# yjh0410/YOLO-Nano

Hardware: AMD Instinct MI355X
Metric: images/sec YOLO-Nano-1.0x 416x416 bs=32 inference (network + decode + NMS + host delivery) (higher is better)
Workload: dtype f32 (split-f16 MFMA x3, fp32 accumulate); 1 GPU; YOLO-Nano-1.0x 416x416 bs=32/GPU fp32 inference, COCO 80-class head + NMS (BASELINE configs[1]); inputs resident in HBM, kept detections delivered to pinned host memory inside the timed region; global_batch=32, parallelism=image-sharded x1, no collective, rccl_ranks=1, launch_mode=eager, streams_per_gpu=4

## Files before the change

include/yolonano_hip.h:

```cpp
#ifndef YOLONANO_HIP_H
#define YOLONANO_HIP_H

#include <stdint.h>

#ifdef __cplusplus
extern "C" {
#endif

typedef struct yn_handle yn_handle;

enum { YN_BACKBONE_0_5X = 0, YN_BACKBONE_1_0X = 1, YN_BACKBONE_1_5X = 2, YN_BACKBONE_2_0X = 3 };
enum { YN_ACT_NONE = 0, YN_ACT_RELU = 1, YN_ACT_LEAKY = 2 };
enum { YN_F32 = 0, YN_F16 = 1 };
enum { YN_STATUS_OK = 0, YN_STATUS_ERROR = 1, YN_STATUS_RANGE = 2 };

typedef struct yn_config {
    int   input_size;
    int   num_classes;
    int   num_anchors;
    float anchors[18];
    int   backbone;
    float conf_thresh;
    float nms_thresh;
    int   diou_nms;
// ... 166 lines not shown
int  yn_train_get_loss_scale(yn_handle* h, float* scale, float* clean_steps);
int  yn_train_set_loss_scale(yn_handle* h, float scale, float clean_steps);
int  yn_allreduce_grads(yn_handle* h, void* nccl_comm);
int  yn_train_forward(yn_handle* h, const float* x_dev, int B, float* head_s8_dev, float* head_s16_dev, float* head_s32_dev);
int  yn_train_skipped_steps(yn_handle* h, int64_t* count_host);
int  yn_train_head_fork(yn_handle* h, int force, int* decision_host);
int  yn_train_precision(yn_handle* h, int dtype);
int  yn_train_graph(yn_handle* h, int enable, int64_t* replays);

int  yn_op_dwconv3x3(yn_handle* h, const float* x, int B, int H, int W, int C, int stride,
                     const float* w, const float* bias, int act, float* y);
int  yn_op_pwconv(yn_handle* h, const float* x, int B, int H, int W, int Cin, int Cout,
                  const float* w, const float* bias, int act, float* y);
int  yn_op_pwconv_shuffle(yn_handle* h, const float* x, const float* pass, int B, int H, int W, int Cin, int Cout,
                          const float* w, const float* bias, int act, float* y);
int  yn_op_conv3x3(yn_handle* h, const float* x, const float* x2, int resample, int B, int H, int W,
                   int Cin, int Cout, const float* w, const float* bias, int act, float* y);
int  yn_op_stem(yn_handle* h, const float* x_nchw, int B, int H, int W, int Cout,
                const float* w, const float* bias, int act, float* y);
int  yn_op_stem_pool(yn_handle* h, const float* x_nchw, int B, int H, int W, int Cout,
                     const float* w, const float* bias, int act, float* y);
int  yn_op_maxpool3x3s2(yn_handle* h, const float* x, int B, int H, int W, int C, float* y);
int  yn_op_shuffle_block(yn_handle* h, const char* block, const float* x, int B, int H, int W, float* y);
int  yn_op_nchw_to_nhwc(yn_handle* h, const float* x, int B, int C, int H, int W, float* y);
int  yn_op_nhwc_to_nchw(yn_handle* h, const float* x, int B, int C, int H, int W, float* y);

int  yn_op_h16_conv(yn_handle* h, int kind, const float* x, int B, int H, int W, int Cin, int gapped, const float* w, const float* bias,
                    int Cout, int stride, const float* dy, float* y, float* dx, float* dw);
int  yn_op_h16_conv2(yn_handle* h, int kind, const float* x, int B, int H, int W, int Cin, int gapped, int x_ld, int x_off,
                     const float* w, const float* bias, int Cout, int stride, const float* dy, int accumulate, int dx_ld, int dx_off,
                     int64_t partial_cap, int stat, const float* y_below, const float* mean, const float* invstd, const float* gamma,
                     const float* beta, int act, float* y, float* dx, float* dw, float* dbias, double* sums_fwd, double* sums_bwd);
int  yn_op_h16_stem(yn_handle* h, const float* x_nchw, int B, int H, int W, const float* w, const float* bias, const float* dy, float* y, float* dw);
int  yn_op_h16_maxpool(yn_handle* h, const float* x, int B, int H, int W, int C, const float* dy, float* y, uint8_t* idx, float* dx);
int  yn_op_h16_stem_pool(yn_handle* h, const float* y, int B, int H, int W, const float* gamma, const float* beta, int act, const float* g1,
                         float* out, uint8_t* idx, float* mean, float* invstd, float* dy, float* dgamma, float* dbeta);
int  yn_op_h16_resample(yn_handle* h, int mode, const float* a, const float* b, float* out, int B, int H, int W, int C);
int  yn_op_h16_gather(yn_handle* h, const float* src, int src_ld, int src_off, int src_cs, int src_half, int src_gap,
                      float* dst, int dst_ld, int dst_off, int dst_cs, int dst_half, int dst_gap, int64_t M, int n, int npad);
int  yn_op_h16_grad_finish(yn_handle* h, float* g, const float* slots, int64_t n, float* state, int update, int global_flag);
int  yn_op_h16_loss(yn_handle* h, const float* head_s8, const float* head_s16, const float* head_s32, const float* target, int B, float scale,
                    float* losses, float* g_s8, float* g_s16, float* g_s32, int* pad_nonzero);
int  yn_op_h16_gemm_stats(yn_handle* h, int kind, const float* x, int B, int H, int W, int Cin, int gapped, const float* w, int Cout,
                          float* y, double* sums_fwd, const float* dy, const float* y_below, const float* mean, const float* invstd,
                          const float* gamma, const float* beta, int act, float* dx, double* sums_bwd);
int  yn_op_h16_bn(yn_handle* h, const float* y, const float* dz, int64_t M, int C, const float* gamma, const float* beta, int act,
// ... 50 lines not shown
```

yolo-nano_amd/capi.py:

```python
import ctypes
import os

import numpy as np
import torch

from . import arch

_HERE = os.path.dirname(os.path.abspath(__file__))
LIB_PATH = os.path.join(_HERE, "libyolonano_hip.so")

_vp = ctypes.c_void_p
_i32, _f32 = ctypes.c_int, ctypes.c_float
_i64p = ctypes.POINTER(ctypes.c_int64)

BACKBONE_ID = {"0.5x": 0, "1.0x": 1, "1.5x": 2, "2.0x": 3}


class YnConfig(ctypes.Structure):
    _fields_ = [("input_size", _i32), ("num_classes", _i32), ("num_anchors", _i32),
                ("anchors", _f32 * 18), ("backbone", _i32), ("conf_thresh", _f32), ("nms_thresh", _f32),
                ("diou_nms", _i32), ("max_batch", _i32), ("device", _i32), ("stream", _vp)]


SIGNATURES = {
# ... 52 lines not shown
    "yn_train_forward": (_i32, [_vp, _vp, _i32, _vp, _vp, _vp]),
    "yn_train_skipped_steps": (_i32, [_vp, _i64p]),
    "yn_train_head_fork": (_i32, [_vp, _i32, ctypes.POINTER(ctypes.c_int)]),
    "yn_train_precision": (_i32, [_vp, _i32]),
    "yn_train_graph": (_i32, [_vp, _i32, _vp]),
    "yn_train_get_loss_scale": (_i32, [_vp, ctypes.POINTER(_f32), ctypes.POINTER(_f32)]),
    "yn_train_set_loss_scale": (_i32, [_vp, _f32, _f32]),
    "yn_make_targets": (_i32, [_vp, _vp, _vp, _i32, _vp, _vp]),
    "yn_preprocess": (_i32, [_vp, _vp, _i32, _i32, _i32, _i32, _i32, _i32, _i32, _vp, _vp, _vp]),
    "yn_preprocess_batch": (_i32, [_vp, _i32, _vp, _vp, _i32, _vp, _vp, _vp]),
    "yn_train_transform_batch": (_i32, [_vp, _i32, _vp, _vp, _vp, _i32, _vp, _vp, _vp]),
    "yn_mosaic_transform_batch": (_i32, [_vp, _i32, _vp, _vp, _vp, _i32, _i32, _vp, _vp, _vp]),
    "yn_nms_merge": (_i32, [_vp, _vp, _vp, _vp, _i32, _i32, _f32, _i32, _vp, _vp, _vp, _vp, _vp]),
    "yn_ema_update": (_i32, [_vp, _vp, _vp, ctypes.c_int64, ctypes.c_double]),
    "yn_sgd_step": (_i32, [_vp, _vp, _vp, _vp, ctypes.c_int64, _f32, _f32, _f32, _f32, _i32]),
    "yn_op_dwconv3x3": (_i32, [_vp, _vp, _i32, _i32, _i32, _i32, _i32, _vp, _vp, _i32, _vp]),
    "yn_op_pwconv": (_i32, [_vp, _vp, _i32, _i32, _i32, _i32, _i32, _vp, _vp, _i32, _vp]),
    "yn_op_pwconv_shuffle": (_i32, [_vp, _vp, _vp, _i32, _i32, _i32, _i32, _i32, _vp, _vp, _i32, _vp]),
    "yn_op_conv3x3": (_i32, [_vp, _vp, _vp, _i32, _i32, _i32, _i32, _i32, _i32, _vp, _vp, _i32, _vp]),
    "yn_op_stem": (_i32, [_vp, _vp, _i32, _i32, _i32, _i32, _vp, _vp, _i32, _vp]),
    "yn_op_stem_pool": (_i32, [_vp, _vp, _i32, _i32, _i32, _i32, _vp, _vp, _i32, _vp]),
    "yn_op_maxpool3x3s2": (_i32, [_vp, _vp, _i32, _i32, _i32, _i32, _vp]),
    "yn_op_shuffle_block": (_i32, [_vp, ctypes.c_char_p, _vp, _i32, _i32, _i32, _vp]),
    "yn_op_nchw_to_nhwc": (_i32, [_vp, _vp, _i32, _i32, _i32, _i32, _vp]),
    "yn_op_nhwc_to_nchw": (_i32, [_vp, _vp, _i32, _i32, _i32, _i32, _vp]),
    "yn_op_h16_conv": (_i32, [_vp, _i32, _vp, _i32, _i32, _i32, _i32, _i32, _vp, _vp, _i32, _i32, _vp, _vp, _vp, _vp]),
    "yn_op_h16_conv2": (_i32, [_vp, _i32, _vp, _i32, _i32, _i32, _i32, _i32, _i32, _i32, _vp, _vp, _i32, _i32, _vp, _i32, _i32, _i32, ctypes.c_int64,
                               _i32, _vp, _vp, _vp, _vp, _vp, _i32, _vp, _vp, _vp, _vp, _vp, _vp]),
    "yn_op_h16_stem": (_i32, [_vp, _vp, _i32, _i32, _i32, _vp, _vp, _vp, _vp, _vp]),
    "yn_op_h16_maxpool": (_i32, [_vp, _vp, _i32, _i32, _i32, _i32, _vp, _vp, _vp, _vp]),
    "yn_op_h16_stem_pool": (_i32, [_vp, _vp, _i32, _i32, _i32, _vp, _vp, _i32, _vp, _vp, _vp, _vp, _vp, _vp, _vp, _vp]),
    "yn_op_h16_resample": (_i32, [_vp, _i32, _vp, _vp, _vp, _i32, _i32, _i32, _i32]),
    "yn_op_h16_gather": (_i32, [_vp, _vp, _i32, _i32, _i32, _i32, _i32, _vp, _i32, _i32, _i32, _i32, _i32, ctypes.c_int64, _i32, _i32]),
    "yn_op_h16_grad_finish": (_i32, [_vp, _vp, _vp, ctypes.c_int64, _vp, _i32, _i32]),
    "yn_op_h16_loss": (_i32, [_vp, _vp, _vp, _vp, _vp, _i32, _f32, _vp, _vp, _vp, _vp, ctypes.POINTER(_i32)]),
    "yn_op_h16_bn2": (_i32, [_vp, _vp, _vp, ctypes.c_int64, _i32, _vp, _vp, _i32, _vp, _vp, _vp, _vp, _vp, _vp]),
    "yn_op_h16_bn": (_i32, [_vp, _vp, _vp, ctypes.c_int64, _i32, _vp, _vp, _i32, _vp, _vp, _vp, _vp]),
    "yn_op_h16_gemm_stats": (_i32, [_vp, _i32, _vp, _i32, _i32, _i32, _i32, _i32, _vp, _i32, _vp, _vp, _vp, _vp, _vp, _vp, _vp, _vp, _i32, _vp, _vp]),
    "yn_op_h16_bn_unit": (_i32, [_vp, _vp, _vp, _vp, ctypes.c_int64, _i32, _vp, _vp, _i32, _vp, _vp, _vp, _vp, _vp]),
    "yn_op_f32_conv": (_i32, [_vp, _i32, _vp, _i32, _i32, _i32, _i32, _i32, _i32, _vp, _vp, _i32, _i32, _i32, ctypes.c_int64, _vp, _i32, _vp, _vp, _vp, _vp]),
    "yn_op_f32_bn": (_i32, [_vp, _vp, ctypes.c_int64, _i32, _vp, _vp, _i32, _i32, _vp, _vp, _vp, _vp, _vp, _vp, _vp, _i32, _i32, _vp, _vp, _vp, _vp]),
    "yn_op_f32_maxpool": (_i32, [_vp, _vp, _i32, _i32, _i32, _i32, _vp, _vp, _vp, _vp]),
    "yn_op_f32_resample": (_i32, [_vp, _i32, _vp, _vp, _vp, _i32, _i32, _i32, _i32]),
    "yn_eval_create": (_i32, [_vp, _i32, ctypes.c_double, ctypes.POINTER(_vp)]),
    "yn_eval_destroy": (None, [_vp]),
    "yn_eval_reset": (_i32, [_vp, _vp]),
# ... 638 lines not shown
        return y

    def op_stem_pool(self, x_nchw, w, bias, act=0):
        B, _, H, W = x_nchw.shape
        Cout = w.shape[0]
        Hc, Wc = (H - 1) // 2 + 1, (W - 1) // 2 + 1
        y = torch.empty((B, (Hc - 1) // 2 + 1, (Wc - 1) // 2 + 1, Cout), dtype=torch.float32, device=x_nchw.device)
        self._ck(self.lib.yn_op_stem_pool(self.h, _ptr(self._in(x_nchw)), B, H, W, Cout, _ptr(self._in(w)),
                                          _ptr(self._in(bias)) if bias is not None else None, act, y.data_ptr()), "yn_op_stem_pool")
        return y

    def op_maxpool(self, x):
        B, H, W, C = x.shape
        y = torch.empty((B, (H - 1) // 2 + 1, (W - 1) // 2 + 1, C), dtype=torch.float32, device=x.device)
        self._ck(self.lib.yn_op_maxpool3x3s2(self.h, _ptr(self._in(x)), B, H, W, C, y.data_ptr()), "yn_op_maxpool3x3s2")
        return y

    def op_shuffle_block(self, block, x, cout, stride):
        B, H, W, _ = x.shape
        y = torch.empty((B, (H - 1) // stride + 1, (W - 1) // stride + 1, cout), dtype=torch.float32, device=x.device)
        self._ck(self.lib.yn_op_shuffle_block(self.h, block.encode(), _ptr(self._in(x)), B, H, W, y.data_ptr()), "yn_op_shuffle_block")
        return y

    def op_h16_conv(self, kind, x, w, bias=None, stride=1, dy=None, gapped=False):
        B, H, W, Cin = x.shape
        Cout = w.shape[0]
        Ho, Wo = (H - 1) // stride + 1, (W - 1) // stride + 1
        y = torch.empty((B, Ho, Wo, Cout), dtype=torch.float32, device=x.device)
        dx = torch.empty_like(x) if dy is not None else None
        dw = torch.empty_like(w) if dy is not None else None
        self._ck(self.lib.yn_op_h16_conv(self.h, int(kind), self._in(x).data_ptr(), B, H, W, Cin, int(bool(gapped)), self._in(w).data_ptr(), _ptr(bias),
                                         Cout, int(stride), _ptr(self._in(dy) if dy is not None else None), y.data_ptr(), _ptr(dx), _ptr(dw)), "yn_op_h16_conv")
        return y, dx, dw

    def op_h16_bn(self, y, gamma, beta, act=0, dz=None):
        M, C = y.shape
        z = torch.empty_like(y)
        dy = torch.empty_like(y) if dz is not None else None
        dg = torch.empty((C,), dtype=torch.float32, device=y.device) if dz is not None else None
        db = torch.empty((C,), dtype=torch.float32, device=y.device) if dz is not None else None
        self._ck(self.lib.yn_op_h16_bn(self.h, self._in(y).data_ptr(), _ptr(self._in(dz) if dz is not None else None), M, C, gamma.data_ptr(), beta.data_ptr(),
                                       int(act), z.data_ptr(), _ptr(dy), _ptr(dg), _ptr(db)), "yn_op_h16_bn")
        return z, dy, dg, db

    def op_h16_bn2(self, y, gamma, beta, act=0, dz=None):
        M, C = y.shape
# ... 278 lines not shown
```

yolo-nano_amd/csrc/kernels_chain.hip:

```cpp
#include "yn_internal.h"
#include "yn_device.h"

#include <cstdlib>

namespace ynk {

template <int WM, int WN, int NT, int V>
__global__ __launch_bounds__(256, 2) void unit_chain_kernel(ChainArgs a)
{
    typedef typename VecT<V>::type vec;
    constexpr int BM = 32 * WM, BN = 32 * NT * WN, KP = 16, BS = BN * 2, B_PER = KP * BN / 512, G = V / 2;
    constexpr int MAXB = (BM * (BN / (2 * G)) + 255) / 256;
    static_assert(WM * WN == 4 && B_PER >= 1, "4 waves");
    extern __shared__ __attribute__((aligned(16))) float uc_smem[];
    const int bf = a.bf, CS = bf + 2, W = a.W, H = a.H, HW = H * W;
    float* T = uc_smem;
    float* Bs = uc_smem + ((BM * CS + 3) & ~3);

    const int t = threadIdx.x, lane = t & 63, wave = t >> 6, l31 = lane & 31, h = lane >> 5;
    const int wm = wave % WM, wn = wave / WM;
    const int m0 = (int)xcd_block(blockIdx.x, gridDim.x) * BM;
    if (m0 >= a.M) return;
    const int nchunks = (bf + 2 * KP - 1) / (2 * KP), kp_total = bf >> 1;

// ... 530 lines not shown
    if (a.Ws2h) {
        if (!dry && launch_unit_pipe(a, s)) return true;
        if (a.Npad == 64 && !v4) YN_UC2(2, 2, 1, 2, 4)
        if (a.Npad == 64 && v4) YN_UC2(2, 2, 1, 4, 4)
        constexpr int small_m = 4096;
        if (a.Npad == 128 && v4 && a.M <= small_m) YN_UC2(1, 4, 1, 4, 4)
        if (a.Npad == 128 && v4) YN_UC2(2, 2, 2, 4, 3)
        if (a.Npad == 256 && v4) YN_UC2(1, 4, 2, 4, 3)
        if (a.Npad == 32 && v4) YN_UC2(4, 1, 1, 4, 4)
        if (a.Npad == 96 && v4) YN_UC2(4, 1, 3, 4, 2)
        return false;
    }
#undef YN_UC2
    const int tiles64 = (a.M + 63) / 64;
    if (a.Npad == 64 && !v4) YN_UC(2, 2, 1, 2)
    if (a.Npad == 64 && v4) YN_UC(2, 2, 1, 4)
    if (a.Npad == 128 && v4) YN_UC(2, 2, 2, 4)
    if (a.Npad == 256 && v4) { if (tiles64 >= 256) YN_UC(2, 2, 4, 4) else YN_UC(1, 4, 2, 4) }
    if (a.Npad == 32 && v4) YN_UC(4, 1, 1, 4)
    if (a.Npad == 96 && v4) YN_UC(4, 1, 3, 4)
#undef YN_UC
    return false;
}
template <int NP, bool RELU>
__global__ __launch_bounds__(256, 2) void down_unit_pipe_kernel(DownArgs a, int tiles)
{
    constexpr int TW = 8, TH = 4, WW = 2 * TW + 1, WH = 2 * TH + 1, NPIX = WW * WH, RT1 = (NPIX + 31) / 32;
    constexpr int BN = 32 * NP, AST1 = 32 + 8, AST2 = BN + 8, NO = TW * TH, NLD = 5, KS2 = 2 * NP;
    extern __shared__ __attribute__((aligned(16))) float du_smem[];
    const int bf = a.bf, CS = bf + 2, cin = a.cin, cq = cin >> 2;
    h16* A1h = reinterpret_cast<h16*>(du_smem);
    h16* A1l = A1h + RT1 * 32 * AST1;
    h16* A2h = A1h;
    h16* A2l = A2h + NO * AST2;
    h16* A3h = A2l + NO * AST2;
    h16* A3l = A3h + NO * AST1;
    float* X32 = du_smem + RT1 * 32 * AST1;
    float* T32 = X32 + RT1 * 32 * cin;
    unsigned char* inside = reinterpret_cast<unsigned char*>(T32 + RT1 * 32 * CS);

    const int t = threadIdx.x, lane = t & 63, wave = __builtin_amdgcn_readfirstlane(t >> 6), l31 = lane & 31, h = lane >> 5;
    const int Ho = a.H >> 1, Wo = a.W >> 1;
    const int tx_n = (Wo + TW - 1) / TW, ty_n = (Ho + TH - 1) / TH, per_img = tx_n * ty_n;
    const int KQ1 = (cin + 7) >> 3, KQ2 = (bf + 7) >> 3;
    const int TL = (tiles + 7) >> 3, GL = (int)(gridDim.x >> 3);
    const int tbase = (int)(blockIdx.x & 7u) * TL;
    int tl = (int)(blockIdx.x >> 3);
    if (tl >= TL || tbase + tl >= tiles) return;
    auto act_pw = [&](float v, int act) { return RELU ? __builtin_fmaxf(v, 0.0f) : apply_act(v, act); };

#ifdef YN_EXP_TIMING
    long long TS[8]; int tsn = 0;
#define YN_TS() if (tsn < 8) TS[tsn++] = __builtin_readcyclecounter()
#else
#define YN_TS()
#endif
    YN_TS();
    const int cp_n = bf >> 1, ppl = 256 / cp_n;
    const int cp = t % cp_n, dpl = t / cp_n, dc = cp * 2;
    const bool dworker = dpl < ppl;
    float2 wd[9], bd = make_float2(0.0f, 0.0f);
#pragma unroll
    for (int k = 0; k < 9; ++k) wd[k] = dworker ? *reinterpret_cast<const float2*>(a.wdw + k * bf + dc) : make_float2(0.0f, 0.0f);
    if (dworker) bd = *reinterpret_cast<const float2*>(a.bdw + dc);
    const int c1_n = cin >> 1, p1_n = 256 / c1_n;
    const int c1 = (t % c1_n) * 2, p1 = t / c1_n;
    constexpr int NI1 = 2;
    float2 w1d[9], b1d;
#pragma unroll
    for (int k = 0; k < 9; ++k) w1d[k] = *reinterpret_cast<const float2*>(a.wdw1 + k * cin + c1);
    b1d = *reinterpret_cast<const float2*>(a.bdw1 + c1);
    const int it0 = 3 - wave;
    const int nt1 = (NP == 2) ? (it0 & 1) : 0;
    const bool pw2_wave = wave < NP, b1_wave = wave >= NP && wave < 2 * NP;
    const int nt2 = pw2_wave ? wave : wave - NP;
    auto frag = [&](const void* Wh_, const void* Wl_, int ks, int KQ, int n, bool use, h16x8& bh, h16x8& bl) {
        const int kq = ks * 2 + h;
        const bool ok = use && kq < KQ;
        const size_t off = ((size_t)(ok ? kq : 0) * BN + (ok ? n : 0)) * 8;
        const unsigned mk = opaque_mask(ok);
        uint4 vh = *reinterpret_cast<const uint4*>(reinterpret_cast<const h16*>(Wh_) + off), vl = *reinterpret_cast<const uint4*>(reinterpret_cast<const h16*>(Wl_) + off);
        vh.x &= mk; vh.y &= mk; vh.z &= mk; vh.w &= mk; vl.x &= mk; vl.y &= mk; vl.z &= mk; vl.w &= mk;
        bh = *reinterpret_cast<h16x8*>(&vh); bl = *reinterpret_cast<h16x8*>(&vl);
    };
    h16x8 g1h[2], g1l[2], g2h[KS2], g2l[KS2];
#pragma unroll
    for (int ks = 0; ks < 2; ++ks) frag(a.W1h, a.W1l, ks, KQ1, nt1 * 32 + l31, true, g1h[ks], g1l[ks]);
#pragma unroll
    for (int ks = 0; ks < KS2; ++ks) {
        const bool use = pw2_wave || (b1_wave && ks < 2);
        frag(pw2_wave ? a.W2h : a.W3h, pw2_wave ? a.W2l : a.W3l, ks, pw2_wave ? KQ2 : KQ1, nt2 * 32 + l31, use, g2h[ks], g2l[ks]);
    }
    const float bias1 = (nt1 * 32 + l31 < bf) ? a.b1[nt1 * 32 + l31] : 0.0f;
    const float bias23 = (nt2 * 32 + l31 < bf && (pw2_wave || b1_wave)) ? (pw2_wave ? a.b2 : a.b3)[nt2 * 32 + l31] : 0.0f;
    const int QR = WW * cq;
    int wpos[NLD], wrel[NLD];
#pragma unroll
    for (int i = 0; i < NLD; ++i) {
        const int e = t + 256 * i;
        const int wy = e / QR, q = e - wy * QR;
        const int wx = q / cq, c4 = (q - wx * cq) * 4;
        wpos[i] = (e < WH * QR) ? (wy | (wx << 8) | (c4 << 16)) : -1;
        wrel[i] = (wy * a.W + wx) * cin + c4;
    }
    float4 pre[NLD];
    unsigned pok = 0;
    const char* xbase = reinterpret_cast<const char*>(a.x);
    auto request = [&](int tile) {
        const int b = tile / per_img, trem = tile - b * per_img;
        const int ty = trem / tx_n, tx = trem - ty * tx_n;
        const int iy0 = 2 * ty * TH - 1, ix0 = 2 * tx * TW - 1;
        const int org = ((b * a.H + iy0) * a.W + ix0) * cin;
        pok = 0;
#pragma unroll
        for (int i = 0; i < NLD; ++i) {
            const int wy = wpos[i] & 0xff, wx = (wpos[i] >> 8) & 0xff;
            const bool ok = wpos[i] >= 0 && (unsigned)(iy0 + wy) < (unsigned)a.H && (unsigned)(ix0 + wx) < (unsigned)a.W;
            pre[i] = *reinterpret_cast<const float4*>(xbase + (unsigned)(ok ? org + wrel[i] : 0) * 4u);
// ... 2 lines not shown
    };
    request(tbase + tl);
    if (t < RT1 * 32 - NPIX) inside[NPIX + t] = 0;
    float amax = 0.0f;
    float* PT = T32;

    auto consume = [&]() {
#pragma unroll
        for (int i = 0; i < NLD; ++i) {
            if (wpos[i] >= 0) {
                const int wy = wpos[i] & 0xff, wx = (wpos[i] >> 8) & 0xff, c4 = (wpos[i] >> 16) & 0xff;
                const int p = wy * WW + wx;
                const float4 v = vmask(pre[i], 0u - ((pok >> i) & 1u));
                *reinterpret_cast<float4*>(X32 + p * cin + c4) = v;
                const float x4[4] = {v.x, v.y, v.z, v.w};
                h16x4 hi, lo;
#pragma unroll
                for (int j = 0; j < 4; ++j) { amax = range_track(amax, x4[j]); hi[j] = (h16)x4[j]; lo[j] = split_lo(x4[j], hi[j]); }
                *reinterpret_cast<h16x4*>(A1h + p * AST1 + c4) = hi;
                *reinterpret_cast<h16x4*>(A1l + p * AST1 + c4) = lo;
                if (c4 == 0) inside[p] = (unsigned char)((pok >> i) & 1u);
            }
        }
        {
            const int ntail = (32 - cin) >> 2;
            for (int i = t; i < RT1 * 32 * ntail; i += 256) {
                const int p = i / ntail, c2 = cin + 4 * (i - p * ntail);
                *reinterpret_cast<uint2*>(A1h + p * AST1 + c2) = make_uint2(0u, 0u);
                *reinterpret_cast<uint2*>(A1l + p * AST1 + c2) = make_uint2(0u, 0u);
            }
        }
    };
    consume();

    for (;;) {
        const int tile = tbase + tl;
        const int b = tile / per_img, trem = tile - b * per_img;
        const int oy0 = (trem / tx_n) * TH, ox0 = (trem % tx_n) * TW;
        __syncthreads();
        YN_TS();
        const bool more = tl + GL < TL && tbase + tl + GL < tiles;
        if (more) request(tbase + tl + GL);

        for (int it = it0; it < RT1 * NP; it += 4) {
            const int rt = it / NP;
            f32x16 acc0, acc1;
#pragma unroll
            for (int k = 0; k < 16; ++k) { acc0[k] = 0.0f; acc1[k] = 0.0f; }
            const h16* Ahb = A1h + (rt * 32 + l31) * AST1 + h * 8;
            const h16* Alb = A1l + (rt * 32 + l31) * AST1 + h * 8;
            int inw[4];
#pragma unroll
            for (int g = 0; g < 4; ++g) inw[g] = *reinterpret_cast<const int*>(inside + rt * 32 + 8 * g + 4 * h);
#pragma unroll
            for (int ks = 0; ks < 2; ++ks) {
                const h16x8 ah = *reinterpret_cast<const h16x8*>(Ahb + ks * 16);
                const h16x8 al = *reinterpret_cast<const h16x8*>(Alb + ks * 16);
                split_mfma(ah, al, &g1h[ks], &g1l[ks], acc0, acc1);
            }
            const int n = nt1 * 32 + l31;
            if (n < bf) {
                float* trow = T32 + (rt * 32 + 4 * h) * CS + n;
#pragma unroll
                for (int r = 0; r < 16; ++r) {
                    const float v = act_pw(split_join(acc0[r], acc1[r]) + bias1, a.act1);
                    trow[((r & 3) + 8 * (r >> 2)) * CS] = __uint_as_float(__float_as_uint(v) & (unsigned)__builtin_amdgcn_sbfe(inw[r >> 2], 8 * (r & 3), 1));
                }
            }
        }
        __syncthreads();
        YN_TS();

        if (p1 < p1_n) {
#pragma unroll
            for (int i = 0; i < NI1; ++i) {
                const int op = p1 + i * p1_n;
                if (op < NO) {
                    const int dy = op / TW, dx = op - dy * TW;
                    float2 acc = b1d;
                    const float* xw = X32 + (2 * dy * WW + 2 * dx) * cin + c1;
#pragma unroll
                    for (int k = 0; k < 9; ++k) vfma(acc, *reinterpret_cast<const float2*>(xw + ((k / 3) * WW + k % 3) * cin), w1d[k]);
                    if (!RELU) acc = vact(acc, a.dw1_act);
                    amax = range_track(range_track(amax, acc.x), acc.y);
                    h16x2 hi, lo;
                    hi[0] = (h16)acc.x; hi[1] = (h16)acc.y;
                    lo[0] = split_lo(acc.x, hi[0]); lo[1] = split_lo(acc.y, hi[1]);
                    *reinterpret_cast<h16x2*>(A3h + op * AST1 + c1) = hi;
                    *reinterpret_cast<h16x2*>(A3l + op * AST1 + c1) = lo;
                }
            }
        }
        {
            const int pad1 = (AST1 - cin) >> 2;
            for (int i = t; i < NO * pad1; i += 256) {
                const int r = i / pad1, c2 = cin + 4 * (i - r * pad1);
                *reinterpret_cast<uint2*>(A3h + r * AST1 + c2) = make_uint2(0u, 0u);
                *reinterpret_cast<uint2*>(A3l + r * AST1 + c2) = make_uint2(0u, 0u);
            }
        }
        if (dworker) {
            for (int op = dpl; op < NO; op += ppl) {
                const int dy = op / TW, dx = op - dy * TW;
                float2 acc = bd;
                const float* yw = T32 + (2 * dy * WW + 2 * dx) * CS + dc;
#pragma unroll
                for (int ky = 0; ky < 3; ++ky)
#pragma unroll
                    for (int kx = 0; kx < 3; ++kx)
                        vfma(acc, *reinterpret_cast<const float2*>(yw + (ky * WW + kx) * CS), wd[ky * 3 + kx]);
                if (!RELU) acc = vact(acc, a.dw_act);
                amax = range_track(range_track(amax, acc.x), acc.y);
                h16x2 hi, lo;
                hi[0] = (h16)acc.x; hi[1] = (h16)acc.y;
                lo[0] = split_lo(acc.x, hi[0]); lo[1] = split_lo(acc.y, hi[1]);
                *reinterpret_cast<h16x2*>(A2h + op * AST2 + dc) = hi;
                *reinterpret_cast<h16x2*>(A2l + op * AST2 + dc) = lo;
            }
        }
        {
            const int padn = (AST2 - bf) >> 1;
            for (int i = t; i < NO * padn; i += 256) {
                const int r = i / padn, c2 = bf + 2 * (i - r * padn);
                *reinterpret_cast<unsigned*>(A2h + r * AST2 + c2) = 0u;
                *reinterpret_cast<unsigned*>(A2l + r * AST2 + c2) = 0u;
            }
        }
        __syncthreads();
        YN_TS();

        f32x16 acc0, acc1;
#pragma unroll
        for (int k = 0; k < 16; ++k) { acc0[k] = 0.0f; acc1[k] = 0.0f; }
        if (b1_wave) {
            const h16* Ahb = A3h + l31 * AST1 + h * 8;
            const h16* Alb = A3l + l31 * AST1 + h * 8;
#pragma unroll
            for (int ks = 0; ks < 2; ++ks) {
                const h16x8 ah = *reinterpret_cast<const h16x8*>(Ahb + ks * 16);
                const h16x8 al = *reinterpret_cast<const h16x8*>(Alb + ks * 16);
                split_mfma(ah, al, &g2h[ks], &g2l[ks], acc0, acc1);
            }
            float* prow = PT + (4 * h) * (BN + 1) + nt2 * 32 + l31;
#pragma unroll
            for (int r = 0; r < 16; ++r)
                prow[((r & 3) + 8 * (r >> 2)) * (BN + 1)] = act_pw(split_join(acc0[r], acc1[r]) + bias23, a.act3);
        }
        if (pw2_wave) {
            const h16* Ahb = A2h + l31 * AST2 + h * 8;
            const h16* Alb = A2l + l31 * AST2 + h * 8;
#pragma unroll
            for (int ks = 0; ks < KS2; ++ks) {
                const h16x8 ah = *reinterpret_cast<const h16x8*>(Ahb + ks * 16);
                const h16x8 al = *reinterpret_cast<const h16x8*>(Alb + ks * 16);
                split_mfma(ah, al, &g2h[ks], &g2l[ks], acc0, acc1);
            }
        }
        __syncthreads();
        if (more) consume();
        if (pw2_wave) {
            const int n = wave * 32 + l31;
            char* obase = reinterpret_cast<char*>(a.out);
            const unsigned lane_off = (unsigned)((((b * Ho + oy0) * Wo + ox0) + 4 * h) * 2 * bf + 2 * n) * 4u;
            const float* prow = PT + (4 * h) * (BN + 1) + n;
            float pv[16];
#pragma unroll
            for (int r = 0; r < 16; ++r) pv[r] = prow[((r & 3) + 8 * (r >> 2)) * (BN + 1)];
#pragma unroll
            for (int r = 0; r < 16; ++r) {
                const int dy = r >> 2, dxu = r & 3;
                if (oy0 + dy < Ho) {
                    if (n < bf && ox0 + dxu + 4 * h < Wo) {
                        const float v = act_pw(split_join(acc0[r], acc1[r]) + bias23, a.act2);
                        *reinterpret_cast<float2*>(obase + (lane_off + (unsigned)((dy * Wo + dxu) * 2 * bf) * 4u)) = make_float2(pv[r], v);
                    }
                }
            }
        }
        YN_TS();
        if (!more) break;
        tl += GL;
    }
    range_report(a.ovf, amax);
#ifdef YN_EXP_TIMING
    if (t == 0 && (blockIdx.x % 61) == 7 && tsn >= 5)
        printf("downpipe blk %d invariants+window %lld gemm1 %lld dw %lld gemm2+store %lld first tile %lld second %lld\n", (int)blockIdx.x, TS[1] - TS[0], TS[2] - TS[1], TS[3] - TS[2],
               TS[4] - TS[3], TS[4] - TS[0], tsn >= 8 ? TS[7] - TS[4] : -1LL);
#endif
#undef YN_TS
}

static size_t down_unit_pipe_lds(int bf, int cin)
{
    return ((size_t)160 * 40 + (size_t)160 * cin + (size_t)160 * (bf + 2)) * sizeof(float) + 160;
}

bool down_unit_covers(const DownArgs& a)
{
    return a.W1h && a.W1l && a.W2h && a.W2l && a.cin <= 32 && !(a.cin & 3) && a.bf <= 64 && !(a.bf & 1) && a.Npad1 == a.Npad2 && a.Npad1 <= 64 &&
           !(a.H & 1) && !(a.W & 1) && a.B > 0 && a.cin >= 16 && (size_t)a.B * a.H * a.W * (size_t)(a.cin > a.bf / 2 ? a.cin : a.bf / 2) < ((size_t)1 << 30) &&
           a.wdw1 && a.bdw1 && a.W3h && a.W3l && a.b3 && a.Npad3 == a.Npad1;
}

void launch_down_unit(const DownArgs& a, hipStream_t s)
{
    const int Ho = a.H >> 1, Wo = a.W >> 1;
    const unsigned tiles = (unsigned)a.B * ((Ho + 3) / 4) * ((Wo + 7) / 8);
    const int NP = a.Npad1 / 32;
    static unsigned long long attr = 0;
    if (attr_pending(attr)) {
        (void)hipFuncSetAttribute(reinterpret_cast<const void*>(down_unit_pipe_kernel<1, true>), hipFuncAttributeMaxDynamicSharedMemorySize, 160 * 1024);
        (void)hipFuncSetAttribute(reinterpret_cast<const void*>(down_unit_pipe_kernel<2, true>), hipFuncAttributeMaxDynamicSharedMemorySize, 160 * 1024);
        (void)hipFuncSetAttribute(reinterpret_cast<const void*>(down_unit_pipe_kernel<1, false>), hipFuncAttributeMaxDynamicSharedMemorySize, 160 * 1024);
        (void)hipFuncSetAttribute(reinterpret_cast<const void*>(down_unit_pipe_kernel<2, false>), hipFuncAttributeMaxDynamicSharedMemorySize, 160 * 1024);
    }
    constexpr unsigned pipe_g = 1024;
    const size_t plds = down_unit_pipe_lds(a.bf, a.cin);
    unsigned g = xcd_grid(tiles);
    if (g > pipe_g) g = pipe_g;
    const bool relu = a.act1 == 1 && a.act2 == 1 && a.act3 == 1 && a.dw_act == 0 && a.dw1_act == 0;
#define YN_DUP(np, rl) { set_last_kernel_name("down_unit_pipe_kernel<" #np "," #rl ">"); hipLaunchKernelGGL((down_unit_pipe_kernel<np, rl>), dim3(g), dim3(256), plds, s, a, (int)tiles); }
    if (NP == 1) { if (relu) YN_DUP(1, true) else YN_DUP(1, false) }
    else         { if (relu) YN_DUP(2, true) else YN_DUP(2, false) }
#undef YN_DUP
}

template <int NT, int D>
__global__ __launch_bounds__(256, NT == 1 ? 3 : 1) void down2_kernel(Down2Args a)
{
    constexpr int BM = 32;
    extern __shared__ __attribute__((aligned(16))) float d2_smem[];
    const int bf = a.bf, cin = a.cin;
    const int KQ2 = (bf + 7) >> 3, KQ1 = (cin + 7) >> 3, PS2 = plane_stride(bf), PS1 = plane_stride(cin);
    const int S2 = (KQ2 + 1) >> 1, S1 = (KQ1 + 1) >> 1, S = S2 + S1;
    const bool chain = a.W1nh != nullptr;
    h16* A2h = reinterpret_cast<h16*>(d2_smem);
    h16* A2l = A2h + BM * PS2;
    h16* A1h = A2l + BM * PS2;
    h16* A1l = A1h + BM * PS1;

    const int t = threadIdx.x, lane = t & 63, wave = t >> 6, l31 = lane & 31, h = lane >> 5;
    const int Ho = (a.H - 1) / 2 + 1, Wo = (a.W - 1) / 2 + 1, HWo = Ho * Wo, Mo = a.B * HWo;
    const int m0 = (int)xcd_block(blockIdx.x, gridDim.x) * BM;
    if (m0 >= Mo) return;
    const int nrows = Mo - m0 < BM ? Mo - m0 : BM;

// ... 369 lines not shown
```

yolo-nano_amd/csrc/yn_api.hip:

```cpp
#include <hip/hip_runtime.h>

#include <dlfcn.h>

#include <cstdarg>
#include <cstdio>
#include <cstring>
#include <map>
#include <mutex>
#include <string>
#include <vector>

#include "../../include/yolonano_hip.h"
#include "yn_internal.h"
#include "yn_h16.h"
#include <stdlib.h>

using namespace ynk;

namespace {

thread_local std::string g_create_error;
std::mutex g_tune_mutex;
std::map<std::vector<int>, int> g_pw_tuned;

// ... 1961 lines not shown
    const int bf = pw1.cout, C = 2 * bf;
    const int Cin = s2 ? pw1.cin : C;
    const int Ho = s2 ? (H - 1) / 2 + 1 : H, Wo = s2 ? (W - 1) / 2 + 1 : W;
    const long Mi = (long)B * H * W, Mo = (long)B * Ho * Wo;
    DevBuf<float> t1, t2, tdw, tb1;
    HIPCHK(h, t1.reserve((size_t)Mi * bf));
    HIPCHK(h, t2.reserve((size_t)Mo * bf));
    if (s2) {
        HIPCHK(h, tdw.reserve((size_t)Mo * Cin));
        HIPCHK(h, tb1.reserve((size_t)Mo * bf));
        run_dw(h, L(h, P + ".b1.dw"), x, Cin, 0, B, H, W, tdw, Cin, 0);
        run_pw(h, L(h, P + ".b1.pw"), tdw, Cin, 0, Mo, tb1, bf, 0, nullptr, 0, 0);
        run_pw(h, pw1, x, Cin, 0, Mi, t1, bf, 0, nullptr, 0, 0);
        run_dw(h, L(h, P + ".b2.dw"), t1, bf, 0, B, H, W, t2, bf, 0);
        run_pw(h, L(h, P + ".b2.pw2"), t2, bf, 0, Mo, y, C, 0, tb1, bf, 0);
    } else {
        run_unit(h, P, x, B, H, W, y, t1, t2);
    }
    HIPCHK(h, hipGetLastError());
    HIPCHK(h, hipStreamSynchronize(h->stream));
    return 0;
}

int yn_op_nchw_to_nhwc(yn_handle* h, const float* x, int B, int C, int H, int W, float* y)
{
    YN_ENTER(h);
    launch_nchw_to_nhwc(x, B, C, H, W, y, h->stream);
    HIPCHK(h, hipGetLastError());
    return 0;
}

int yn_op_nhwc_to_nchw(yn_handle* h, const float* x, int B, int C, int H, int W, float* y)
{
    YN_ENTER(h);
    launch_nhwc_to_nchw(x, B, C, H, W, y, h->stream);
    HIPCHK(h, hipGetLastError());
    return 0;
}

int yn_profile_enable(yn_handle* h, int enable)
{
    YN_ENTER(h);
    h->profiling = enable != 0;
    h->prof.clear();
    h->event_next = 0;
    return 0;
// ... 576 lines not shown
```

Measured before the change: 49720 images/s.

## Specialize down-unit pipe kernel on channel widths with staged output writes

Templates the fused stride-2 down-unit kernel on input width and branch width so loop bounds, padding loops and load counts become compile-time constants. It prefetches LDS fragments two iterations ahead in the first pointwise stage and batches the depthwise loads before the FMAs. Both branch outputs are now interleaved in LDS and written as coalesced float4 stores. Coverage is narrowed to cin=24 with branch width 24 or 58, and a test entry point for the unit is added.

Result: faster. 50600 images/s, median of 6 (+1.8%).

```diff
diff --git a/include/yolonano_hip.h b/include/yolonano_hip.h
--- a/include/yolonano_hip.h
+++ b/include/yolonano_hip.h
@@ -212,6 +212,7 @@
                      const float* w, const float* bias, int act, float* y);
 int  yn_op_maxpool3x3s2(yn_handle* h, const float* x, int B, int H, int W, int C, float* y);
 int  yn_op_shuffle_block(yn_handle* h, const char* block, const float* x, int B, int H, int W, float* y);
+int  yn_op_down_unit(yn_handle* h, const char* block, const float* x, int B, int H, int W, float* y);
 int  yn_op_nchw_to_nhwc(yn_handle* h, const float* x, int B, int C, int H, int W, float* y);
 int  yn_op_nhwc_to_nchw(yn_handle* h, const float* x, int B, int C, int H, int W, float* y);
 
diff --git a/yolo-nano_amd/capi.py b/yolo-nano_amd/capi.py
--- a/yolo-nano_amd/capi.py
+++ b/yolo-nano_amd/capi.py
@@ -98,6 +98,7 @@
     "yn_op_stem_pool": (_i32, [_vp, _vp, _i32, _i32, _i32, _i32, _vp, _vp, _i32, _vp]),
     "yn_op_maxpool3x3s2": (_i32, [_vp, _vp, _i32, _i32, _i32, _i32, _vp]),
     "yn_op_shuffle_block": (_i32, [_vp, ctypes.c_char_p, _vp, _i32, _i32, _i32, _vp]),
+    "yn_op_down_unit": (_i32, [_vp, ctypes.c_char_p, _vp, _i32, _i32, _i32, _vp]),
     "yn_op_nchw_to_nhwc": (_i32, [_vp, _vp, _i32, _i32, _i32, _i32, _vp]),
     "yn_op_nhwc_to_nchw": (_i32, [_vp, _vp, _i32, _i32, _i32, _i32, _vp]),
     "yn_op_h16_conv": (_i32, [_vp, _i32, _vp, _i32, _i32, _i32, _i32, _i32, _vp, _vp, _i32, _i32, _vp, _vp, _vp, _vp]),
@@ -782,6 +783,12 @@
         self._ck(self.lib.yn_op_shuffle_block(self.h, block.encode(), _ptr(self._in(x)), B, H, W, y.data_ptr()), "yn_op_shuffle_block")
         return y
 
+    def op_down_unit(self, block, x, cout):
+        B, H, W, _ = x.shape
+        y = torch.empty((B, H // 2, W // 2, cout), dtype=torch.float32, device=x.device)
+        self._ck(self.lib.yn_op_down_unit(self.h, block.encode(), _ptr(self._in(x)), B, H, W, y.data_ptr()), "yn_op_down_unit")
+        return y
+
     def op_h16_conv(self, kind, x, w, bias=None, stride=1, dy=None, gapped=False):
         B, H, W, Cin = x.shape
         Cout = w.shape[0]
diff --git a/yolo-nano_amd/csrc/kernels_chain.hip b/yolo-nano_amd/csrc/kernels_chain.hip
--- a/yolo-nano_amd/csrc/kernels_chain.hip
+++ b/yolo-nano_amd/csrc/kernels_chain.hip
@@ -576,13 +576,16 @@
 #undef YN_UC
     return false;
 }
-template <int NP, bool RELU>
+template <int CIN, int BF, bool RELU>
 __global__ __launch_bounds__(256, 2) void down_unit_pipe_kernel(DownArgs a, int tiles)
 {
+    constexpr int NP = (BF + 31) / 32;
     constexpr int TW = 8, TH = 4, WW = 2 * TW + 1, WH = 2 * TH + 1, NPIX = WW * WH, RT1 = (NPIX + 31) / 32;
-    constexpr int BN = 32 * NP, AST1 = 32 + 8, AST2 = BN + 8, NO = TW * TH, NLD = 5, KS2 = 2 * NP;
+    constexpr int BN = 32 * NP, AST1 = 32 + 8, AST2 = BN + 8, NO = TW * TH, KS2 = 2 * NP;
+    constexpr int bf = BF, CS = bf + 2, cin = CIN, cq = cin >> 2;
+    constexpr int NLD = (WH * WW * cq + 255) / 256;
+    static_assert(CIN >= 16 && CIN <= 32 && !(CIN & 3) && BF <= 64 && !(BF & 1) && BF / 2 <= 256, "down_unit_covers");
     extern __shared__ __attribute__((aligned(16))) float du_smem[];
-    const int bf = a.bf, CS = bf + 2, cin = a.cin, cq = cin >> 2;
     h16* A1h = reinterpret_cast<h16*>(du_smem);
     h16* A1l = A1h + RT1 * 32 * AST1;
     h16* A2h = A1h;
@@ -596,7 +599,7 @@
     const int t = threadIdx.x, lane = t & 63, wave = __builtin_amdgcn_readfirstlane(t >> 6), l31 = lane & 31, h = lane >> 5;
     const int Ho = a.H >> 1, Wo = a.W >> 1;
     const int tx_n = (Wo + TW - 1) / TW, ty_n = (Ho + TH - 1) / TH, per_img = tx_n * ty_n;
-    const int KQ1 = (cin + 7) >> 3, KQ2 = (bf + 7) >> 3;
+    constexpr int KQ1 = (cin + 7) >> 3, KQ2 = (bf + 7) >> 3;
     const int TL = (tiles + 7) >> 3, GL = (int)(gridDim.x >> 3);
     const int tbase = (int)(blockIdx.x & 7u) * TL;
     int tl = (int)(blockIdx.x >> 3);
@@ -610,16 +613,16 @@
 #define YN_TS()
 #endif
     YN_TS();
-    const int cp_n = bf >> 1, ppl = 256 / cp_n;
+    constexpr int cp_n = bf >> 1, ppl = 256 / cp_n, NI2 = (NO + ppl - 1) / ppl;
     const int cp = t % cp_n, dpl = t / cp_n, dc = cp * 2;
     const bool dworker = dpl < ppl;
     float2 wd[9], bd = make_float2(0.0f, 0.0f);
 #pragma unroll
     for (int k = 0; k < 9; ++k) wd[k] = dworker ? *reinterpret_cast<const float2*>(a.wdw + k * bf + dc) : make_float2(0.0f, 0.0f);
     if (dworker) bd = *reinterpret_cast<const float2*>(a.bdw + dc);
-    const int c1_n = cin >> 1, p1_n = 256 / c1_n;
+    constexpr int c1_n = cin >> 1, p1_n = 256 / c1_n;
     const int c1 = (t % c1_n) * 2, p1 = t / c1_n;
-    constexpr int NI1 = 2;
+    constexpr int NI1 = (NO + p1_n - 1) / p1_n;
     float2 w1d[9], b1d;
 #pragma unroll
     for (int k = 0; k < 9; ++k) w1d[k] = *reinterpret_cast<const float2*>(a.wdw1 + k * cin + c1);
@@ -647,7 +650,7 @@
     }
     const float bias1 = (nt1 * 32 + l31 < bf) ? a.b1[nt1 * 32 + l31] : 0.0f;
     const float bias23 = (nt2 * 32 + l31 < bf && (pw2_wave || b1_wave)) ? (pw2_wave ? a.b2 : a.b3)[nt2 * 32 + l31] : 0.0f;
-    const int QR = WW * cq;
+    constexpr int QR = WW * cq;
     int wpos[NLD], wrel[NLD];
 #pragma unroll
     for (int i = 0; i < NLD; ++i) {
@@ -696,9 +699,12 @@
                 if (c4 == 0) inside[p] = (unsigned char)((pok >> i) & 1u);
             }
         }
-        {
-            const int ntail = (32 - cin) >> 2;
-            for (int i = t; i < RT1 * 32 * ntail; i += 256) {
+        if constexpr (cin < 32) {
+            constexpr int ntail = (32 - cin) >> 2;
+#pragma unroll
+            for (int i0 = 0; i0 < RT1 * 32 * ntail; i0 += 256) {
+                const int i = i0 + t;
+                if (i0 + 256 > RT1 * 32 * ntail && i >= RT1 * 32 * ntail) break;
                 const int p = i / ntail, c2 = cin + 4 * (i - p * ntail);
                 *reinterpret_cast<uint2*>(A1h + p * AST1 + c2) = make_uint2(0u, 0u);
                 *reinterpret_cast<uint2*>(A1l + p * AST1 + c2) = make_uint2(0u, 0u);
@@ -716,85 +722,125 @@
         const bool more = tl + GL < TL && tbase + tl + GL < tiles;
         if (more) request(tbase + tl + GL);
 
-        for (int it = it0; it < RT1 * NP; it += 4) {
-            const int rt = it / NP;
-            f32x16 acc0, acc1;
-#pragma unroll
-            for (int k = 0; k < 16; ++k) { acc0[k] = 0.0f; acc1[k] = 0.0f; }
-            const h16* Ahb = A1h + (rt * 32 + l31) * AST1 + h * 8;
-            const h16* Alb = A1l + (rt * 32 + l31) * AST1 + h * 8;
-            int inw[4];
-#pragma unroll
-            for (int g = 0; g < 4; ++g) inw[g] = *reinterpret_cast<const int*>(inside + rt * 32 + 8 * g + 4 * h);
-#pragma unroll
-            for (int ks = 0; ks < 2; ++ks) {
-                const h16x8 ah = *reinterpret_cast<const h16x8*>(Ahb + ks * 16);
-                const h16x8 al = *reinterpret_cast<const h16x8*>(Alb + ks * 16);
-                split_mfma(ah, al, &g1h[ks], &g1l[ks], acc0, acc1);
-            }
-            const int n = nt1 * 32 + l31;
-            if (n < bf) {
-                float* trow = T32 + (rt * 32 + 4 * h) * CS + n;
-#pragma unroll
-                for (int r = 0; r < 16; ++r) {
-                    const float v = act_pw(split_join(acc0[r], acc1[r]) + bias1, a.act1);
-                    trow[((r & 3) + 8 * (r >> 2)) * CS] = __uint_as_float(__float_as_uint(v) & (unsigned)__builtin_amdgcn_sbfe(inw[r >> 2], 8 * (r & 3), 1));
+        {
+            constexpr int NITEMS = RT1 * NP, NFULL = NITEMS / 4, NIT1 = (NITEMS + 3) / 4;
+            const bool last_ok = it0 + 4 * NFULL < NITEMS;
+            h16x8 fah[NIT1][2], fal[NIT1][2];
+            int inw[NIT1][4];
+            auto reads = [&](int j) {
+                const int rt = (j < NFULL || last_ok) ? (it0 + 4 * j) / NP : 0;
+                const h16* Ahb = A1h + (rt * 32 + l31) * AST1 + h * 8;
+                const h16* Alb = A1l + (rt * 32 + l31) * AST1 + h * 8;
+#pragma unroll
+                for (int ks = 0; ks < 2; ++ks) {
+                    fah[j][ks] = *reinterpret_cast<const h16x8*>(Ahb + ks * 16);
+                    fal[j][ks] = *reinterpret_cast<const h16x8*>(Alb + ks * 16);
+                }
+#pragma unroll
+                for (int g = 0; g < 4; ++g) inw[j][g] = *reinterpret_cast<const int*>(inside + rt * 32 + 8 * g + 4 * h);
+            };
+            reads(0);
+            if (NIT1 > 1) reads(1);
+#pragma unroll
+            for (int j = 0; j < NIT1; ++j) {
+                if (j + 2 < NIT1) reads(j + 2);
+                if (j < NFULL || last_ok) {
+                    f32x16 acc0, acc1;
+#pragma unroll
+                    for (int k = 0; k < 16; ++k) { acc0[k] = 0.0f; acc1[k] = 0.0f; }
+#pragma unroll
+                    for (int ks = 0; ks < 2; ++ks) split_mfma(fah[j][ks], fal[j][ks], &g1h[ks], &g1l[ks], acc0, acc1);
+                    const int rt = (it0 + 4 * j) / NP;
+                    const int n = nt1 * 32 + l31;
+                    if (n < bf) {
+                        float* trow = T32 + (rt * 32 + 4 * h) * CS + n;
+#pragma unroll
+                        for (int r = 0; r < 16; ++r) {
+                            const float v = act_pw(split_join(acc0[r], acc1[r]) + bias1, a.act1);
+                            trow[((r & 3) + 8 * (r >> 2)) * CS] = __uint_as_float(__float_as_uint(v) & (unsigned)__builtin_amdgcn_sbfe(inw[j][r >> 2], 8 * (r & 3), 1));
+                        }
+                    }
                 }
             }
         }
         __syncthreads();
         YN_TS();
 
-        if (p1 < p1_n) {
+        {
+            float2 xv[NI1][9], acc[NI1];
+#pragma unroll
+            for (int i = 0; i < NI1; ++i) {
+                const int op = p1 + i * p1_n, opc = op < NO ? op : 0;
+                const int dy = opc / TW, dx = opc - dy * TW;
+                const float* xw = X32 + (2 * dy * WW + 2 * dx) * cin + c1;
+#pragma unroll
+                for (int k = 0; k < 9; ++k) xv[i][k] = *reinterpret_cast<const float2*>(xw + ((k / 3) * WW + k % 3) * cin);
+                acc[i] = b1d;
+            }
+#pragma unroll
+            for (int k = 0; k < 9; ++k)
+#pragma unroll
+                for (int i = 0; i < NI1; ++i) vfma(acc[i], xv[i][k], w1d[k]);
 #pragma unroll
             for (int i = 0; i < NI1; ++i) {
                 const int op = p1 + i * p1_n;
-                if (op < NO) {
-                    const int dy = op / TW, dx = op - dy * TW;
-                    float2 acc = b1d;
-                    const float* xw = X32 + (2 * dy * WW + 2 * dx) * cin + c1;
-#pragma unroll
-                    for (int k = 0; k < 9; ++k) vfma(acc, *reinterpret_cast<const float2*>(xw + ((k / 3) * WW + k % 3) * cin), w1d[k]);
-                    if (!RELU) acc = vact(acc, a.dw1_act);
-                    amax = range_track(range_track(amax, acc.x), acc.y);
+                if (p1 < p1_n && op < NO) {
+                    if (!RELU) acc[i] = vact(acc[i], a.dw1_act);
+                    amax = range_track(range_track(amax, acc[i].x), acc[i].y);
                     h16x2 hi, lo;
-                    hi[0] = (h16)acc.x; hi[1] = (h16)acc.y;
-                    lo[0] = split_lo(acc.x, hi[0]); lo[1] = split_lo(acc.y, hi[1]);
+                    hi[0] = (h16)acc[i].x; hi[1] = (h16)acc[i].y;
+                    lo[0] = split_lo(acc[i].x, hi[0]); lo[1] = split_lo(acc[i].y, hi[1]);
                     *reinterpret_cast<h16x2*>(A3h + op * AST1 + c1) = hi;
                     *reinterpret_cast<h16x2*>(A3l + op * AST1 + c1) = lo;
                 }
             }
         }
         {
-            const int pad1 = (AST1 - cin) >> 2;
-            for (int i = t; i < NO * pad1; i += 256) {
+            constexpr int pad1 = (AST1 - cin) >> 2;
+#pragma unroll
+            for (int i0 = 0; i0 < NO * pad1; i0 += 256) {
+                const int i = i0 + t;
+                if (i0 + 256 > NO * pad1 && i >= NO * pad1) break;
                 const int r = i / pad1, c2 = cin + 4 * (i - r * pad1);
                 *reinterpret_cast<uint2*>(A3h + r * AST1 + c2) = make_uint2(0u, 0u);
                 *reinterpret_cast<uint2*>(A3l + r * AST1 + c2) = make_uint2(0u, 0u);
             }
         }
-        if (dworker) {
-            for (int op = dpl; op < NO; op += ppl) {
-                const int dy = op / TW, dx = op - dy * TW;
-                float2 acc = bd;
+        {
+            float2 yv[NI2][9], acc[NI2];
+#pragma unroll
+            for (int i = 0; i < NI2; ++i) {
+                const int op = dpl + i * ppl, opc = op < NO ? op : 0;
+                const int dy = opc / TW, dx = opc - dy * TW;
                 const float* yw = T32 + (2 * dy * WW + 2 * dx) * CS + dc;
 #pragma unroll
-                for (int ky = 0; ky < 3; ++ky)
-#pragma unroll
-                    for (int kx = 0; kx < 3; ++kx)
-                        vfma(acc, *reinterpret_cast<const float2*>(yw + (ky * WW + kx) * CS), wd[ky * 3 + kx]);
-                if (!RELU) acc = vact(acc, a.dw_act);
-                amax = range_track(range_track(amax, acc.x), acc.y);
-                h16x2 hi, lo;
-                hi[0] = (h16)acc.x; hi[1] = (h16)acc.y;
-                lo[0] = split_lo(acc.x, hi[0]); lo[1] = split_lo(acc.y, hi[1]);
-                *reinterpret_cast<h16x2*>(A2h + op * AST2 + dc) = hi;
-                *reinterpret_cast<h16x2*>(A2l + op * AST2 + dc) = lo;
+                for (int k = 0; k < 9; ++k) yv[i][k] = *reinterpret_cast<const float2*>(yw + ((k / 3) * WW + k % 3) * CS);
+                acc[i] = bd;
+            }
+#pragma unroll
+            for (int k = 0; k < 9; ++k)
+#pragma unroll
+                for (int i = 0; i < NI2; ++i) vfma(acc[i], yv[i][k], wd[k]);
+#pragma unroll
+            for (int i = 0; i < NI2; ++i) {
+                const int op = dpl + i * ppl;
+                if (dworker && op < NO) {
+                    if (!RELU) acc[i] = vact(acc[i], a.dw_act);
+                    amax = range_track(range_track(amax, acc[i].x), acc[i].y);
+                    h16x2 hi, lo;
+                    hi[0] = (h16)acc[i].x; hi[1] = (h16)acc[i].y;
+                    lo[0] = split_lo(acc[i].x, hi[0]); lo[1] = split_lo(acc[i].y, hi[1]);
+                    *reinterpret_cast<h16x2*>(A2h + op * AST2 + dc) = hi;
+                    *reinterpret_cast<h16x2*>(A2l + op * AST2 + dc) = lo;
+                }
             }
         }
         {
-            const int padn = (AST2 - bf) >> 1;
-            for (int i = t; i < NO * padn; i += 256) {
+            constexpr int padn = (AST2 - bf) >> 1;
+#pragma unroll
+            for (int i0 = 0; i0 < NO * padn; i0 += 256) {
+                const int i = i0 + t;
+                if (i0 + 256 > NO * padn && i >= NO * padn) break;
                 const int r = i / padn, c2 = bf + 2 * (i - r * padn);
                 *reinterpret_cast<unsigned*>(A2h + r * AST2 + c2) = 0u;
                 *reinterpret_cast<unsigned*>(A2l + r * AST2 + c2) = 0u;
@@ -806,6 +852,7 @@
         f32x16 acc0, acc1;
 #pragma unroll
         for (int k = 0; k < 16; ++k) { acc0[k] = 0.0f; acc1[k] = 0.0f; }
+        constexpr int PS = 2 * bf;
         if (b1_wave) {
             const h16* Ahb = A3h + l31 * AST1 + h * 8;
             const h16* Alb = A3l + l31 * AST1 + h * 8;
@@ -815,10 +862,6 @@
                 const h16x8 al = *reinterpret_cast<const h16x8*>(Alb + ks * 16);
                 split_mfma(ah, al, &g2h[ks], &g2l[ks], acc0, acc1);
             }
-            float* prow = PT + (4 * h) * (BN + 1) + nt2 * 32 + l31;
-#pragma unroll
-            for (int r = 0; r < 16; ++r)
-                prow[((r & 3) + 8 * (r >> 2)) * (BN + 1)] = act_pw(split_join(acc0[r], acc1[r]) + bias23, a.act3);
         }
         if (pw2_wave) {
             const h16* Ahb = A2h + l31 * AST2 + h * 8;
@@ -830,25 +873,31 @@
                 split_mfma(ah, al, &g2h[ks], &g2l[ks], acc0, acc1);
             }
         }
+        if ((pw2_wave || b1_wave) && nt2 * 32 + l31 < bf) {
+            float* prow = PT + (4 * h) * PS + 2 * (nt2 * 32 + l31) + (pw2_wave ? 1 : 0);
+            const int act23 = pw2_wave ? a.act2 : a.act3;
+#pragma unroll
+            for (int r = 0; r < 16; ++r)
+                prow[((r & 3) + 8 * (r >> 2)) * PS] = act_pw(split_join(acc0[r], acc1[r]) + bias23, act23);
+        }
         __syncthreads();
         if (more) consume();
-        if (pw2_wave) {
-            const int n = wave * 32 + l31;
+        {
             char* obase = reinterpret_cast<char*>(a.out);
-            const unsigned lane_off = (unsigned)((((b * Ho + oy0) * Wo + ox0) + 4 * h) * 2 * bf + 2 * n) * 4u;
-            const float* prow = PT + (4 * h) * (BN + 1) + n;
-            float pv[16];
-#pragma unroll
-            for (int r = 0; r < 16; ++r) pv[r] = prow[((r & 3) + 8 * (r >> 2)) * (BN + 1)];
-#pragma unroll
-            for (int r = 0; r < 16; ++r) {
-                const int dy = r >> 2, dxu = r & 3;
-                if (oy0 + dy < Ho) {
-                    if (n < bf && ox0 + dxu + 4 * h < Wo) {
-                        const float v = act_pw(split_join(acc0[r], acc1[r]) + bias23, a.act2);
-                        *reinterpret_cast<float2*>(obase + (lane_off + (unsigned)((dy * Wo + dxu) * 2 * bf) * 4u)) = make_float2(pv[r], v);
-                    }
-                }
+            const unsigned tile_off = (unsigned)(((b * Ho + oy0) * Wo + ox0) * 2 * bf) * 4u;
+            constexpr int PQ = bf / 2, RQ = TW * PQ, NST = (TH * RQ + 255) / 256;
+            float4 ov[NST];
+#pragma unroll
+            for (int i = 0; i < NST; ++i) {
+                const int e = t + 256 * i;
+                ov[i] = *reinterpret_cast<const float4*>(PT + (e < TH * RQ ? e : 0) * 4);
+            }
+#pragma unroll
+            for (int i = 0; i < NST; ++i) {
+                const int e = t + 256 * i;
+                const int dy = e / RQ, q = e - dy * RQ, dx = q / PQ;
+                if (e < TH * RQ && oy0 + dy < Ho && ox0 + dx < Wo)
+                    *reinterpret_cast<float4*>(obase + (tile_off + (unsigned)(dy * Wo * 2 * bf) * 4u + (unsigned)q * 16u)) = ov[i];
             }
         }
         YN_TS();
@@ -871,8 +920,9 @@
 
 bool down_unit_covers(const DownArgs& a)
 {
-    return a.W1h && a.W1l && a.W2h && a.W2l && a.cin <= 32 && !(a.cin & 3) && a.bf <= 64 && !(a.bf & 1) && a.Npad1 == a.Npad2 && a.Npad1 <= 64 &&
-           !(a.H & 1) && !(a.W & 1) && a.B > 0 && a.cin >= 16 && (size_t)a.B * a.H * a.W * (size_t)(a.cin > a.bf / 2 ? a.cin : a.bf / 2) < ((size_t)1 << 30) &&
+    const bool widths = a.cin == 24 && (a.bf == 58 || a.bf == 24);
+    return widths && a.W1h && a.W1l && a.W2h && a.W2l && a.Npad1 == a.Npad2 && a.Npad1 == 32 * ((a.bf + 31) / 32) &&
+           !(a.H & 1) && !(a.W & 1) && a.B > 0 && (size_t)a.B * a.H * a.W * (size_t)(a.cin > a.bf / 2 ? a.cin : a.bf / 2) < ((size_t)1 << 30) &&
            a.wdw1 && a.bdw1 && a.W3h && a.W3l && a.b3 && a.Npad3 == a.Npad1;
 }
 
@@ -880,22 +930,21 @@
 {
     const int Ho = a.H >> 1, Wo = a.W >> 1;
     const unsigned tiles = (unsigned)a.B * ((Ho + 3) / 4) * ((Wo + 7) / 8);
-    const int NP = a.Npad1 / 32;
     static unsigned long long attr = 0;
     if (attr_pending(attr)) {
-        (void)hipFuncSetAttribute(reinterpret_cast<const void*>(down_unit_pipe_kernel<1, true>), hipFuncAttributeMaxDynamicSharedMemorySize, 160 * 1024);
-        (void)hipFuncSetAttribute(reinterpret_cast<const void*>(down_unit_pipe_kernel<2, true>), hipFuncAttributeMaxDynamicSharedMemorySize, 160 * 1024);
-        (void)hipFuncSetAttribute(reinterpret_cast<const void*>(down_unit_pipe_kernel<1, false>), hipFuncAttributeMaxDynamicSharedMemorySize, 160 * 1024);
-        (void)hipFuncSetAttribute(reinterpret_cast<const void*>(down_unit_pipe_kernel<2, false>), hipFuncAttributeMaxDynamicSharedMemorySize, 160 * 1024);
+        (void)hipFuncSetAttribute(reinterpret_cast<const void*>(down_unit_pipe_kernel<24, 24, true>), hipFuncAttributeMaxDynamicSharedMemorySize, 160 * 1024);
+        (void)hipFuncSetAttribute(reinterpret_cast<const void*>(down_unit_pipe_kernel<24, 58, true>), hipFuncAttributeMaxDynamicSharedMemorySize, 160 * 1024);
+        (void)hipFuncSetAttribute(reinterpret_cast<const void*>(down_unit_pipe_kernel<24, 24, false>), hipFuncAttributeMaxDynamicSharedMemorySize, 160 * 1024);
+        (void)hipFuncSetAttribute(reinterpret_cast<const void*>(down_unit_pipe_kernel<24, 58, false>), hipFuncAttributeMaxDynamicSharedMemorySize, 160 * 1024);
     }
     constexpr unsigned pipe_g = 1024;
     const size_t plds = down_unit_pipe_lds(a.bf, a.cin);
     unsigned g = xcd_grid(tiles);
     if (g > pipe_g) g = pipe_g;
     const bool relu = a.act1 == 1 && a.act2 == 1 && a.act3 == 1 && a.dw_act == 0 && a.dw1_act == 0;
-#define YN_DUP(np, rl) { set_last_kernel_name("down_unit_pipe_kernel<" #np "," #rl ">"); hipLaunchKernelGGL((down_unit_pipe_kernel<np, rl>), dim3(g), dim3(256), plds, s, a, (int)tiles); }
-    if (NP == 1) { if (relu) YN_DUP(1, true) else YN_DUP(1, false) }
-    else         { if (relu) YN_DUP(2, true) else YN_DUP(2, false) }
+#define YN_DUP(ci, bw, rl) { set_last_kernel_name("down_unit_pipe_kernel<" #ci "," #bw "," #rl ">"); hipLaunchKernelGGL((down_unit_pipe_kernel<ci, bw, rl>), dim3(g), dim3(256), plds, s, a, (int)tiles); }
+    if (a.bf == 24) { if (relu) YN_DUP(24, 24, true) else YN_DUP(24, 24, false) }
+    else            { if (relu) YN_DUP(24, 58, true) else YN_DUP(24, 58, false) }
 #undef YN_DUP
 }
 
diff --git a/yolo-nano_amd/csrc/yn_api.hip b/yolo-nano_amd/csrc/yn_api.hip
--- a/yolo-nano_amd/csrc/yn_api.hip
+++ b/yolo-nano_amd/csrc/yn_api.hip
@@ -2007,6 +2007,35 @@
     return 0;
 }
 
+int yn_op_down_unit(yn_handle* h, const char* block, const float* x, int B, int H, int W, float* y)
+{
+    YN_ENTER(h);
+    if (!h->folded) return fail(h, "yn_op_down_unit before yn_fold_bn");
+    h->cur = h->stream;
+    const std::string P = block;
+    if (!h->by_name.count(P + ".b2.pw1") || !h->by_name.count(P + ".b1.dw")) return fail(h, "'%s' is not a stride-2 block", block);
+    const Layer &lp1 = L(h, P + ".b2.pw1"), &ldw = L(h, P + ".b2.dw"), &lp2 = L(h, P + ".b2.pw2"), &l1d = L(h, P + ".b1.dw"), &l1p = L(h, P + ".b1.pw");
+    const int bf = lp1.cout, Cin = lp1.cin;
+    DownArgs d{};
+    d.x = x; d.cin = Cin;
+    d.W1h = lp1.ws_hi; d.W1l = lp1.ws_lo; d.b1 = lp1.b_packed; d.act1 = lp1.act; d.Npad1 = lp1.Npad;
+    d.wdw = ldw.w_packed; d.bdw = ldw.b_packed; d.dw_act = ldw.act;
+    d.W2h = lp2.ws_hi; d.W2l = lp2.ws_lo; d.b2 = lp2.b_packed; d.act2 = lp2.act; d.Npad2 = lp2.Npad;
+    d.wdw1 = l1d.w_packed; d.bdw1 = l1d.b_packed; d.dw1_act = l1d.act;
+    d.W3h = l1p.ws_hi; d.W3l = l1p.ws_lo; d.b3 = l1p.b_packed; d.act3 = l1p.act; d.Npad3 = l1p.Npad;
+    d.out = y; d.B = B; d.H = H; d.W = W; d.bf = bf;
+    d.ovf = h->range_flags ? h->range_flags + 1 : nullptr;
+    if (exact(h) || lp2.cin != bf || lp2.cout != bf || ldw.stride != 2 || l1d.stride != 2 || l1d.cout != Cin || l1p.cin != Cin || l1p.cout != bf || !down_unit_covers(d))
+        return fail(h, "yn_op_down_unit: down_unit_pipe_kernel does not cover '%s' at %d x %d x %d (cin %d, branch width %d)", block, B, H, W, Cin, bf);
+    {
+        Bracket br(h, P + ".unit", 0.0, 0.0);
+        launch_down_unit(d, h->cur);
+    }
+    HIPCHK(h, hipGetLastError());
+    HIPCHK(h, hipStreamSynchronize(h->stream));
+    return 0;
+}
+
 int yn_op_nchw_to_nhwc(yn_handle* h, const float* x, int B, int C, int H, int W, float* y)
 {
     YN_ENTER(h);
```
